# wangze22/StableDiffusion-PyTorch

Hardware: AMD Instinct MI355X
Metric: DDPM train steps/sec (cond-UNet, CelebHQ-256 latents, B=32) at 1/2/4/8 MI355X (higher is better)
Workload: dtype bf16; 1 GPU; cond-UNet celebhq_text_image_cond training step; model=cond-UNet 118.5M, global_batch=32, per_gpu_batch=32, parallelism=dp1

## Files before the change

### include/sdmi.h

```cpp
#ifndef SDMI_H
#define SDMI_H
#include <stdint.h>
#include <stddef.h>

#ifdef __cplusplus
extern "C" {
#endif

typedef void* sdmi_stream_t;

enum {
  SDMI_A_ROWMAJOR = 0,
  SDMI_A_CONV = 1,
  SDMI_A_COLMAJOR = 2
};
enum {
  SDMI_B_NK = 0,
  SDMI_B_KN = 1,
  SDMI_B_KN_CONV = 2
};

typedef struct sdmi_conv_geom {
  int ih, iw, cin, ldx;
  int kh, kw;
  int oh, ow;
  int sy, sx, oy0, ox0;
} sdmi_conv_geom;

typedef struct sdmi_gemm_desc {
  int m, n, k;
  int a_mode, b_mode;
  const void* a; int lda;
  const void* b; int ldb;
  sdmi_conv_geom geom;
  void* c; int ldc; int c_f32;
  const float* bias;
  const void* rowbias;
  int rb_ld, rb_div;
  const void* resid; int ldr;
  float alpha;
  int act;
  int remap, r_gh, r_gw, r_oh, r_ow, r_sy, r_sx, r_oy, r_ox;
  int perm, p_cin, p_taps, p_cvalid;
  int m_store, n_store;
  const void* a2; int lda2; int k_split;
  const float* bias2;
  int rb_mod;
  const void* aux; int ld_aux;
  int splits_hint;
  int tile_n_hint;
  float* sum_out;
  float* sum_out2;
  void* gsum_out;
  int gsum_ld;
  int sum_group;
  int variant_hint;
  const void* gn_x; int gn_ldx;
  const float* gn_tab;
  float* gn_part;
  int gn_P, gn_rb, gn_silu;
} sdmi_gemm_desc;

int sdmi_gemm_kernel_info(const sdmi_gemm_desc* d, int* variant, int* tile_n);
int sdmi_gemm_plan(const sdmi_gemm_desc* d, int* splits, size_t* workspace_bytes);
int sdmi_gemm(const sdmi_gemm_desc* d, void* workspace, size_t workspace_bytes, sdmi_stream_t stream);

#define SDMI_GEMM_GROUP_MAX 8
int sdmi_gemm_grouped_plan(const sdmi_gemm_desc* d, int ngroups, int* splits, size_t* workspace_bytes);
int sdmi_gemm_grouped(const sdmi_gemm_desc* d, int ngroups, void* workspace, size_t workspace_bytes,
                      sdmi_stream_t stream);

int sdmi_attn_fwd(const void* q, int ldq, const void* k, int ldk, const void* v, int ldv, void* out, int ldo,
                  float* lse, int B, int H, int N, int S, int d, sdmi_stream_t stream);
int sdmi_attn_bwd(const void* q, int ldq, const void* k, int ldk, const void* v, int ldv, const void* o, int ldo,
                  const void* dout, int lddo, const float* lse, float* delta_ws, void* dq, int lddq, void* dk,
                  int lddk, void* dv, int lddv, int B, int H, int N, int S, int d, sdmi_stream_t stream);
size_t sdmi_attn_bwd_workspace(int B, int H, int N, int S, int d);
int sdmi_attn_bwd_fused(const void* q, int ldq, const void* k, int ldk, const void* v, int ldv, const void* o, int ldo,
                        const void* dout, int lddo, const float* lse, float* delta_ws, void* ws, size_t ws_bytes,
                        void* dq, int lddq, void* dk, int lddk, void* dv, int lddv, int B, int H, int N, int S, int d,
                        sdmi_stream_t stream);

size_t sdmi_chan_reduce_workspace(int B, int P, int C);
int sdmi_gn_stats(const void* x, int ldx, int B, int P, int C, int G, float eps, const float* gamma, const float* beta,
                  float* ws, float* table, sdmi_stream_t stream);
int sdmi_gn_fwd(const void* x, int ldx, void* y, int ldy, int B, int P, int C, int G, float eps, const float* gamma,
                const float* beta, int silu, float* ws, float* table, sdmi_stream_t stream);
int sdmi_gn_apply(const void* x, int ldx, void* y, int ldy, const float* table, int B, int P, int C, int silu,
                  sdmi_stream_t stream);
int sdmi_gn_bwd(const void* x, int ldx, const void* dy, int lddy, void* dx, int lddx, const float* table,
                const float* gamma, int B, int P, int C, int G, int silu, float* ws, float* table2_ws, float* dgamma,
                float* dbeta, const void* addend, int ldadd, sdmi_stream_t stream);
int sdmi_gn_bwd_part(const void* x, int ldx, const void* dy, int lddy, void* dx, int lddx, const float* table,
                     const float* gamma, int B, int P, int C, int G, int silu, const float* part, int rb, float* ws,
                     float* dgamma, float* dbeta, const void* addend, int ldadd, sdmi_stream_t stream);

int sdmi_gn_bwd_rows(const void* x, int ldx, const void* dy, int lddy, void* dx, int lddx, const float* table,
                     const float* gamma, int B, int P, int C, int G, int silu, float* ws, float* table2_ws, float* rows,
                     const void* addend, int ldadd, sdmi_stream_t stream);
int sdmi_gn_bwd_part_rows(const void* x, int ldx, const void* dy, int lddy, void* dx, int lddx, const float* table,
                          const float* gamma, int B, int P, int C, int G, int silu, const float* part, int rb, float* ws,
                          float* rows, const void* addend, int ldadd, sdmi_stream_t stream);
int sdmi_gn_rows_sum(const float* rows, int B, int C, float* dgamma, float* dbeta, sdmi_stream_t stream);
#define SDMI_GN_ROWS_GROUP_MAX 16
typedef struct {
  const float* rows;
  float* dgamma;
  float* dbeta;
  int B, C;
} sdmi_gn_rows_job;
int sdmi_gn_rows_sum_grouped(const sdmi_gn_rows_job* jobs, int njobs, sdmi_stream_t stream);


int sdmi_chan_sum(const void* dy, int lddy, int B, int P, int C, float* ws, void* per_bc, int ld_bc, float* per_c,
                  float* per_c2, int c_store, sdmi_stream_t stream);

int sdmi_prep_input(const float* x, int B, int cx, int H, int W, const float* mask, int cmi, int MH, int MW,
                    const float* wcond, int cmo, void* out, int cpad, const float* keep, sdmi_stream_t stream);
int sdmi_cond_wgrad(const void* dxin, int ld, int cx, int B, int H, int W, const float* mask, int cmi, int MH, int MW,
                    int cmo, float* dw, const float* keep, sdmi_stream_t stream);
int sdmi_prep_input_cmap(const float* x, int B, int cx, int H, int W, const unsigned char* cmap, int cmi, int MH,
                         int MW, const float* wcond, int cmo, void* out, int cpad, const float* keep,
                         sdmi_stream_t stream);
int sdmi_cond_wgrad_cmap(const void* dxin, int ld, int cx, int B, int H, int W, const unsigned char* cmap, int cmi,
                         int MH, int MW, int cmo, float* dw, const float* keep, sdmi_stream_t stream);
int sdmi_nhwc_to_nchw(const void* src, int src_f32, int ld, int B, int C, int HW, float* dst, sdmi_stream_t stream);
int sdmi_nchw_to_nhwc_bf16(const float* src, int B, int C, int HW, void* dst, int ld, sdmi_stream_t stream);
int sdmi_add_noise(const float* x0, const float* eps, const long long* t, const float* sqrt_abar,
                   const float* sqrt_one_minus_abar, int B, long long per_sample, float* out, sdmi_stream_t stream);
size_t sdmi_mse_workspace(void);
int sdmi_mse(const float* pred, int ld, const float* target, int B, int C, int HW, float gscale,
             const float* gscale_dev, void* grad, float* ws, float* loss, sdmi_stream_t stream);
int sdmi_time_embedding(const long long* t, int tstride, int B, int dim, void* out, int ld, float* out_f32,
                        sdmi_stream_t stream);
int sdmi_silu(const void* x, const void* dy, void* y, long long n, sdmi_stream_t stream);
int sdmi_relu(const float* x, const float* dy, float* y, long long n, sdmi_stream_t stream);
int sdmi_copy_slice(const void* src, int lds, void* dst, int ldd, long long P, int C, int accumulate,
                    sdmi_stream_t stream);

int sdmi_ln_chunk_rows(int N);
int sdmi_ln_mod_fwd(const void* x, int ldx, const void* v, int ldv, const void* gate, void* xo, int ldxo,
                    const void* shift, const void* scale, int ld_mod, void* y, int ldy, float* mean, float* rstd,
                    int rows, int C, int N, float eps, int x_f32, sdmi_stream_t stream);
int sdmi_ln_mod_bwd(const void* x, int ldx, const float* mean, const float* rstd, const void* dy, int lddy,
                    const void* scale, int ld_mod, const void* dres, int lddres, void* dx, int lddx, float* psh,
                    float* psc, int ws_ld, const void* gate, const void* v, int ldv, void* dv, int lddv, float* pg,
                    int rows, int C, int N, int x_f32, void* dx16, int ld16, sdmi_stream_t stream);
int sdmi_mod_finalize(const float* ws, int B, int chunks, int ws_ld, int W, void* out, int ldo, sdmi_stream_t stream);
int sdmi_tokens_to_nchw(const void* src, int src_f32, int ld, int B, int C, int H, int W, int p, float* dst,
                        sdmi_stream_t stream);
int sdmi_nchw_to_tokens_bf16(const float* src, int B, int C, int H, int W, int p, void* dst, int ld,
                             sdmi_stream_t stream);
int sdmi_mse_patch(const float* pred, int ld, const float* target, int B, int C, int H, int W, int p, float gscale,
                   const float* gscale_dev, void* grad, float* ws, float* loss, sdmi_stream_t stream);

size_t sdmi_vq_workspace(long long pixels);
size_t sdmi_vq_bwd_workspace(void);
int sdmi_vq_bwd(const void* dzin, int ld_dzin, const float* zq, const float* w_post, const float* xq, const long long* idx,
                const float* codebook, int K, const float* z_enc, int ldz, const float* w_pre, int B, int HW, int C,
                float commitment_beta, float codebook_weight, void* dz_enc, int ld_out, float* ws, float* dw_post,
                float* db_post, float* dw_pre, float* db_pre, float* demb, const float* dzq_add, const float* loss_w,
                sdmi_stream_t stream);
int sdmi_vq_quantize(const float* z, int ldz, const float* w, const float* b, const float* codebook, int K, int B,
                     int HW, int C, float* zq, long long* idx, float* xq, float* ws, float* loss, sdmi_stream_t stream);
int sdmi_pointwise_in(const float* z, int B, int C, int HW, const float* w, const float* b, int cout, void* out,
                      int ld, sdmi_stream_t stream);

int sdmi_lpips_prep(const float* in0, int in0_nhwc, const float* in1, int in1_nhwc, int B, int H, int W,
                    const float* shift, const float* scale, int normalize, void* out, sdmi_stream_t stream);
int sdmi_lpips_image_grad(const void* d, int B, int H, int W, const float* scale, int normalize, float* out_nchw,
                          void* acc_nhwc, const float* mse_pred, const float* mse_target, sdmi_stream_t stream);
int sdmi_maxpool2_fwd(const void* x, int N, int H, int W, int C, void* y, sdmi_stream_t stream);
int sdmi_maxpool2_bwd(const void* x, const void* dy, int N, int H, int W, int C, void* dx, sdmi_stream_t stream);
size_t sdmi_lpips_dist_workspace(int B, int P, int C);
int sdmi_lpips_dist_fwd(const void* f, int ld, const float* w, int B, int P, int C, float* rn, float* ws, int accumulate,
                        float* val, sdmi_stream_t stream);
int sdmi_lpips_dist_bwd(const void* f, int ld, const float* w, const float* rn, const float* g, float gscale, int B,
                        int P, int C, int side, const void* addend, int ld_add, void* dy, int ld_dy,
                        sdmi_stream_t stream);
int sdmi_lpips_mean(const float* val, int B, float scale, float* out, sdmi_stream_t stream);

int sdmi_ddpm_prev(const float* xt, const float* eps, const float* z, long long n, long long* t_dev, const float* betas,
                   const float* alphas, const float* abar, const float* s1m, float* prev, float* x0, int decrement_t,
                   sdmi_stream_t stream);
int sdmi_ddim_prev(const float* xt, const float* eps, const float* noise, long long n, float alpha_t, float alpha_prev,
                   float eta, float* out, sdmi_stream_t stream);
int sdmi_ddim_prev_dev(const float* xt, const float* eps, const float* noise, long long n, const long long* ts,
                       const long long* tp, long long* idx, long long* t_dev, const float* abar, float eta, float* out,
                       int advance, sdmi_stream_t stream);
int sdmi_affine_step(const float* x, const float* eps, const float* z, long long n, float c1, float c2, float var,
                     float* out, sdmi_stream_t stream);
int sdmi_cfg_combine(const float* eps_cond, const float* eps_uncond, long long n, float scale, float* out,
                     sdmi_stream_t stream);
int sdmi_cfg_combine_nhwc(const void* pred, int src_f32, int ld, int B, int C, int HW, float scale, float* dst,
                          sdmi_stream_t stream);
int sdmi_ddpm_prev_dup(const float* xt, const float* eps, const float* z, long long n, long long* t_dev,
                       const float* betas, const float* alphas, const float* abar, const float* s1m, float* prev,
                       float* prev2, float* x0, int decrement_t, sdmi_stream_t stream);
int sdmi_ddim_prev_dev_dup(const float* xt, const float* eps, const float* noise, long long n, const long long* ts,
                           const long long* tp, long long* idx, long long* t_dev, const float* abar, float eta,
                           float* out, float* out2, int advance, sdmi_stream_t stream);

int sdmi_randn(float* out, long long n, unsigned long long seed, unsigned long long* offset_dev, int advance,
               sdmi_stream_t stream);

int sdmi_step_draw(float* noise, long long n, long long* t, int B, int T, const float* text, const float* empty,
                   float* txt, long long row_elems, float p_text, float* keep, float p_keep, unsigned long long seed,
                   unsigned long long offset, sdmi_stream_t stream);

typedef struct sdmi_pack_desc {
  const float* src;
  void* dst;
  long long so, si, skh, skw;
  int O, I, Ipad, KH, KW, kh_off, kh_mul, kw_off, kw_mul;
  int dst_ld;
} sdmi_pack_desc;
int sdmi_pack_chunk(void);
int sdmi_pack_weights(const sdmi_pack_desc* descs_dev, const void* bmap_dev, int nblocks, sdmi_stream_t stream);

typedef struct sdmi_tpack_desc {
  const void* src;
  void* dst;
  int O, I, taps;
  int src_ld, src_tap, dst_ld, dst_tap;
  signed char smap[16];
} sdmi_tpack_desc;
int sdmi_pack_transpose(const sdmi_tpack_desc* descs_dev, const void* bmap_dev, int nblocks, sdmi_stream_t stream);

size_t sdmi_optim_workspace(void);
int sdmi_clip_unscale(const float* grads, long long n, float max_norm, float* state, float* ws, int growth_interval,
                      int skip_if_loss_nonfinite, float grad_div, sdmi_stream_t stream);
size_t sdmi_optim_workspace_for(long long n);
int sdmi_clip_unscale_ws(const float* grads, long long n, float max_norm, float* state, float* ws, size_t ws_bytes,
                         int growth_interval, int skip_if_loss_nonfinite, float grad_div, sdmi_stream_t stream);
int sdmi_loss_flag(const float* src, float* dst, int mode, sdmi_stream_t stream);
int sdmi_clip_finalize(const float* partial, int n, float max_norm, float* state, int growth_interval,
                       int skip_if_loss_nonfinite, float grad_div, sdmi_stream_t stream);
int sdmi_adam_ema(float* params, const float* grads, float* m, float* v, float* ema, long long n, const float* state,
                  float lr, float b1, float b2, float eps, float ema_decay, float ema_alpha, sdmi_stream_t stream);
int sdmi_adam_ema_bf16(float* params, const float* grads, float* m, float* v, float* ema, long long n,
                       const float* state, float lr, float b1, float b2, float eps, float ema_decay, float ema_alpha,
                       void* params_bf16, sdmi_stream_t stream);
int sdmi_cast_bf16(const float* src, void* dst, long long n, sdmi_stream_t stream);

int sdmi_resize_nearest(const float* in, int BC, int IH, int IW, float* out, int OH, int OW, sdmi_stream_t stream);
int sdmi_chan_copy(const float* src, int src_c, int src_c0, float* dst, int dst_c, int dst_c0, int B, int C,
                   long long P, sdmi_stream_t stream);
int sdmi_modulate_fwd(const float* x, const float* r, const float* s, const float* t, int ls, float alpha, float* y,
                      int B, int N, int C, sdmi_stream_t stream);
int sdmi_modulate_bwd(const float* x, const float* dy, const float* s, int ls, float alpha, float* dx, float* ds,
                      float* dt, int B, int N, int C, sdmi_stream_t stream);
int sdmi_attn_map(const float* q, int ldq, const float* k, int ldk, int B, int H, int N, int S, int d, float scaling,
                  int average, float* out, sdmi_stream_t stream);


int sdmi_plan_begin(void);
int sdmi_plan_end(void** plan);
int sdmi_plan_recording(void);
int sdmi_plan_note_event(void* event, sdmi_stream_t stream);
int sdmi_plan_note_wait(sdmi_stream_t stream, void* event);
int sdmi_plan_note_callout(int id);
int sdmi_plan_info(const void* plan, int* ops, int* launches);
int sdmi_plan_replay(void* plan, int start, int* callout, int* next);
int sdmi_plan_destroy(void* plan);
int sdmi_plan_op_info(const void* plan, int i, int* kind, const char** name, int* grid, int* block, int* shmem);
int sdmi_plan_op_stream(const void* plan, int i, sdmi_stream_t* stream);
int sdmi_plan_time_op(void* plan, int i, int warm, int iters, float* us);

int sdmi_comm_load(const char* rccl_path);
int sdmi_comm_unique_id(unsigned char* id);
int sdmi_comm_init(const unsigned char* id, int nranks, int rank, void** comm);
int sdmi_allreduce(void* comm, void* buf, long long count, int dtype, sdmi_stream_t stream);
int sdmi_comm_destroy(void* comm);

#ifdef __cplusplus
}
#endif
#endif
```

### stablediffusion-pytorch_amd/csrc/plan.hip

```cpp
#include <cstring>
#include <memory>
#include <new>
#include <vector>

#include "../../include/sdmi.h"
#include "launch.h"

namespace sdmi_rt {

void* g_recording = nullptr;

namespace {

enum OpKind { OP_LAUNCH = 0, OP_EVENT = 1, OP_WAIT = 2, OP_CALLOUT = 3, OP_ALLREDUCE = 4 };

struct alignas(16) Chunk16 {
  unsigned char b[16];
};

struct Op {
  int kind;
  const void* fn = nullptr;
  dim3 grid, block;
  unsigned shmem = 0;
  hipStream_t stream = nullptr;
  hipEvent_t event = nullptr;
  int callout = -1;
  void* comm = nullptr;
  void* buf = nullptr;
  size_t count = 0;
  int dtype = 0;
  std::vector<Chunk16> args;
  std::vector<unsigned> offs;
};

struct Plan {
  std::vector<Op> ops;
  int launches = 0;
  std::vector<void*> scratch;
};

}

void record_launch(const void* fn, dim3 grid, dim3 block, unsigned shmem, hipStream_t stream, const void* args,
                   size_t bytes, const unsigned* offsets, int nargs) {
  Plan* p = (Plan*)g_recording;
  Op op;
  op.kind = OP_LAUNCH;
  op.fn = fn;
  op.grid = grid;
  op.block = block;
  op.shmem = shmem;
  op.stream = stream;
  op.args.resize((bytes + 15) / 16);
  if (bytes) memcpy(op.args.data(), args, bytes);
  op.offs.assign(offsets, offsets + nargs);
  if ((int)p->scratch.size() < nargs) p->scratch.resize(nargs);
  p->ops.push_back(std::move(op));
  ++p->launches;
}

void record_allreduce(void* comm, void* buf, size_t count, int dtype, hipStream_t stream) {
  Plan* p = (Plan*)g_recording;
  Op op;
  op.kind = OP_ALLREDUCE;
  op.comm = comm;
  op.buf = buf;
  op.count = count;
  op.dtype = dtype;
  op.stream = stream;
  p->ops.push_back(std::move(op));
}

}

using sdmi_rt::Plan;

extern "C" int sdmi_plan_begin(void) {
  if (sdmi_rt::g_recording) return -1;
  sdmi_rt::g_recording = new (std::nothrow) Plan();
  return sdmi_rt::g_recording ? 0 : -2;
}

extern "C" int sdmi_plan_end(void** plan) {
  if (!plan || !sdmi_rt::g_recording) return -1;
  *plan = sdmi_rt::g_recording;
  sdmi_rt::g_recording = nullptr;
  return 0;
}

extern "C" int sdmi_plan_recording(void) { return sdmi_rt::g_recording != nullptr; }

extern "C" int sdmi_plan_note_event(void* event, sdmi_stream_t stream) {
  Plan* p = (Plan*)sdmi_rt::g_recording;
  if (!p) return 0;
  if (!event) return -1;
  sdmi_rt::Op op;
  op.kind = sdmi_rt::OP_EVENT;
  op.event = (hipEvent_t)event;
  op.stream = (hipStream_t)stream;
  p->ops.push_back(std::move(op));
  return 0;
}

extern "C" int sdmi_plan_note_wait(sdmi_stream_t stream, void* event) {
  Plan* p = (Plan*)sdmi_rt::g_recording;
  if (!p) return 0;
  if (!event) return -1;
  sdmi_rt::Op op;
  op.kind = sdmi_rt::OP_WAIT;
  op.event = (hipEvent_t)event;
  op.stream = (hipStream_t)stream;
  p->ops.push_back(std::move(op));
  return 0;
}

extern "C" int sdmi_plan_note_callout(int id) {
  Plan* p = (Plan*)sdmi_rt::g_recording;
  if (!p) return 0;
  sdmi_rt::Op op;
  op.kind = sdmi_rt::OP_CALLOUT;
  op.callout = id;
  p->ops.push_back(std::move(op));
  return 0;
}

extern "C" int sdmi_plan_info(const void* plan, int* ops, int* launches) {
  const Plan* p = (const Plan*)plan;
  if (!p) return -1;
  if (ops) *ops = (int)p->ops.size();
  if (launches) *launches = p->launches;
  return 0;
}

extern "C" int sdmi_plan_replay(void* plan, int start, int* callout, int* next) {
  Plan* p = (Plan*)plan;
  if (!p || start < 0 || !callout || !next) return -1;
  void** ptrs = p->scratch.data();
  const int n = (int)p->ops.size();
  for (int i = start; i < n; ++i) {
    const sdmi_rt::Op& op = p->ops[i];
    hipError_t e = hipSuccess;
    switch (op.kind) {
      case sdmi_rt::OP_LAUNCH: {
        const unsigned char* base = (const unsigned char*)op.args.data();
        for (size_t a = 0; a < op.offs.size(); ++a) ptrs[a] = (void*)(base + op.offs[a]);
        e = hipLaunchKernel(op.fn, op.grid, op.block, ptrs, op.shmem, op.stream);
        break;
      }
      case sdmi_rt::OP_EVENT: e = hipEventRecord(op.event, op.stream); break;
      case sdmi_rt::OP_WAIT: e = hipStreamWaitEvent(op.stream, op.event, 0); break;
      case sdmi_rt::OP_ALLREDUCE: {
        const int rc = sdmi_rt::issue_allreduce(op.comm, op.buf, op.count, op.dtype, op.stream);
        if (rc != 0) {
          *callout = -1;
          *next = i;
          return rc;
        }
        break;
      }
      default:
        *callout = op.callout;
        *next = i + 1;
        return 0;
    }
    if (e != hipSuccess) {
      *callout = -1;
      *next = i;
      return (int)e;
    }
  }
  *callout = -1;
  *next = n;
  return 0;
}

extern "C" int sdmi_plan_op_stream(const void* plan, int i, sdmi_stream_t* stream) {
  const Plan* p = (const Plan*)plan;
  if (!p || i < 0 || i >= (int)p->ops.size() || !stream) return -1;
  *stream = (sdmi_stream_t)p->ops[i].stream;
  return 0;
}

extern "C" int sdmi_plan_op_info(const void* plan, int i, int* kind, const char** name, int* grid, int* block,
                                 int* shmem) {
  const Plan* p = (const Plan*)plan;
  if (!p || i < 0 || i >= (int)p->ops.size()) return -1;
  const sdmi_rt::Op& op = p->ops[i];
  if (kind) *kind = op.kind;
  if (name) *name = op.kind == sdmi_rt::OP_LAUNCH ? hipKernelNameRefByPtr(op.fn, op.stream) : nullptr;
  if (grid) {
    grid[0] = (int)op.grid.x;
    grid[1] = (int)op.grid.y;
    grid[2] = (int)op.grid.z;
  }
  if (block) *block = (int)(op.block.x * op.block.y * op.block.z);
  if (shmem) *shmem = (int)op.shmem;
  return 0;
}

extern "C" int sdmi_plan_time_op(void* plan, int i, int warm, int iters, float* us) {
  Plan* p = (Plan*)plan;
  if (!p || i < 0 || i >= (int)p->ops.size() || iters < 1 || !us) return -1;
  const sdmi_rt::Op& op = p->ops[i];
  if (op.kind != sdmi_rt::OP_LAUNCH) return -2;
  void** ptrs = p->scratch.data();
  const unsigned char* base = (const unsigned char*)op.args.data();
  for (size_t a = 0; a < op.offs.size(); ++a) ptrs[a] = (void*)(base + op.offs[a]);
  hipEvent_t e0, e1;
  if (hipEventCreate(&e0) != hipSuccess) return -3;
  if (hipEventCreate(&e1) != hipSuccess) return -3;
  hipError_t e = hipSuccess;
  for (int w = 0; w < warm && e == hipSuccess; ++w) e = hipLaunchKernel(op.fn, op.grid, op.block, ptrs, op.shmem, op.stream);
  if (e == hipSuccess) e = hipEventRecord(e0, op.stream);
  for (int r = 0; r < iters && e == hipSuccess; ++r) e = hipLaunchKernel(op.fn, op.grid, op.block, ptrs, op.shmem, op.stream);
  if (e == hipSuccess) e = hipEventRecord(e1, op.stream);
  if (e == hipSuccess) e = hipEventSynchronize(e1);
  float ms = 0.f;
  if (e == hipSuccess) e = hipEventElapsedTime(&ms, e0, e1);
  (void)hipEventDestroy(e0);
  (void)hipEventDestroy(e1);
  if (e != hipSuccess) return (int)e;
  *us = ms * 1000.f / (float)iters;
  return 0;
}

extern "C" int sdmi_plan_destroy(void* plan) {
  delete (Plan*)plan;
  return 0;
}
```

### stablediffusion-pytorch_amd/sdmi/_lib.py

```python
import ctypes
import os

_HERE = os.path.dirname(os.path.abspath(__file__))
DEFAULT_LIB_PATH = os.path.join(_HERE, "libsdmi.so")
LIB_PATH = os.environ.get("SDMI_LIB_PATH") or DEFAULT_LIB_PATH

A_ROWMAJOR, A_CONV, A_COLMAJOR = 0, 1, 2
B_NK, B_KN, B_KN_CONV = 0, 1, 2


class ConvGeom(ctypes.Structure):
    _fields_ = [(n, ctypes.c_int) for n in
                ("ih", "iw", "cin", "ldx", "kh", "kw", "oh", "ow", "sy", "sx", "oy0", "ox0")]


class GemmDesc(ctypes.Structure):
    _fields_ = [
        ("m", ctypes.c_int), ("n", ctypes.c_int), ("k", ctypes.c_int),
        ("a_mode", ctypes.c_int), ("b_mode", ctypes.c_int),
        ("a", ctypes.c_void_p), ("lda", ctypes.c_int),
        ("b", ctypes.c_void_p), ("ldb", ctypes.c_int),
        ("geom", ConvGeom),
        ("c", ctypes.c_void_p), ("ldc", ctypes.c_int), ("c_f32", ctypes.c_int),
        ("bias", ctypes.c_void_p),
        ("rowbias", ctypes.c_void_p), ("rb_ld", ctypes.c_int), ("rb_div", ctypes.c_int),
        ("resid", ctypes.c_void_p), ("ldr", ctypes.c_int),
        ("alpha", ctypes.c_float),
        ("act", ctypes.c_int),
        ("remap", ctypes.c_int), ("r_gh", ctypes.c_int), ("r_gw", ctypes.c_int),
        ("r_oh", ctypes.c_int), ("r_ow", ctypes.c_int), ("r_sy", ctypes.c_int), ("r_sx", ctypes.c_int),
        ("r_oy", ctypes.c_int), ("r_ox", ctypes.c_int),
        ("perm", ctypes.c_int), ("p_cin", ctypes.c_int), ("p_taps", ctypes.c_int), ("p_cvalid", ctypes.c_int),
        ("m_store", ctypes.c_int), ("n_store", ctypes.c_int),
        ("a2", ctypes.c_void_p), ("lda2", ctypes.c_int), ("k_split", ctypes.c_int),
        ("bias2", ctypes.c_void_p),
        ("rb_mod", ctypes.c_int),
        ("aux", ctypes.c_void_p), ("ld_aux", ctypes.c_int),
        ("splits_hint", ctypes.c_int),
        ("tile_n_hint", ctypes.c_int),
        ("sum_out", ctypes.c_void_p), ("sum_out2", ctypes.c_void_p), ("gsum_out", ctypes.c_void_p),
        ("gsum_ld", ctypes.c_int), ("sum_group", ctypes.c_int),
        ("variant_hint", ctypes.c_int),
        ("gn_x", ctypes.c_void_p), ("gn_ldx", ctypes.c_int),
        ("gn_tab", ctypes.c_void_p),
        ("gn_part", ctypes.c_void_p),
        ("gn_P", ctypes.c_int), ("gn_rb", ctypes.c_int), ("gn_silu", ctypes.c_int),
    ]


_lib = None

_P, _I, _F, _L = ctypes.c_void_p, ctypes.c_int, ctypes.c_float, ctypes.c_longlong
_SZ = ctypes.c_size_t


class GnRowsJob(ctypes.Structure):
    _fields_ = [("rows", ctypes.c_void_p), ("dgamma", ctypes.c_void_p), ("dbeta", ctypes.c_void_p),
                ("B", ctypes.c_int), ("C", ctypes.c_int)]


GN_ROWS_GROUP_MAX = 16


class TPackDesc(ctypes.Structure):
    _fields_ = [("src", ctypes.c_void_p), ("dst", ctypes.c_void_p)] + [(n, ctypes.c_int) for n in (
        "O", "I", "taps", "src_ld", "src_tap", "dst_ld", "dst_tap")] + [("smap", ctypes.c_byte * 16)]


class PackDesc(ctypes.Structure):
    _fields_ = [("src", ctypes.c_void_p), ("dst", ctypes.c_void_p),
                ("so", ctypes.c_longlong), ("si", ctypes.c_longlong), ("skh", ctypes.c_longlong),
                ("skw", ctypes.c_longlong)] + [(n, ctypes.c_int) for n in
                                                ("O", "I", "Ipad", "KH", "KW", "kh_off", "kh_mul", "kw_off", "kw_mul",
                                                 "dst_ld")]


SIGNATURES = {
    "sdmi_gemm_plan": ([ctypes.POINTER(GemmDesc), ctypes.POINTER(ctypes.c_int), ctypes.POINTER(ctypes.c_size_t)], _I),
    "sdmi_gemm": ([ctypes.POINTER(GemmDesc), _P, _SZ, _P], _I),
    "sdmi_gemm_grouped_plan": ([ctypes.POINTER(GemmDesc), _I, ctypes.POINTER(ctypes.c_int),
                                ctypes.POINTER(ctypes.c_size_t)], _I),
    "sdmi_gemm_grouped": ([ctypes.POINTER(GemmDesc), _I, _P, _SZ, _P], _I),
    "sdmi_gemm_kernel_info": ([ctypes.POINTER(GemmDesc), ctypes.POINTER(ctypes.c_int), ctypes.POINTER(ctypes.c_int)],
                              _I),
    "sdmi_attn_fwd": ([_P, _I, _P, _I, _P, _I, _P, _I, _P, _I, _I, _I, _I, _I, _P], _I),
    "sdmi_attn_bwd": ([_P, _I, _P, _I, _P, _I, _P, _I, _P, _I, _P, _P, _P, _I, _P, _I, _P, _I,
                       _I, _I, _I, _I, _I, _P], _I),
    "sdmi_attn_bwd_workspace": ([_I, _I, _I, _I, _I], _SZ),
    "sdmi_attn_bwd_fused": ([_P, _I, _P, _I, _P, _I, _P, _I, _P, _I, _P, _P, _P, _SZ, _P, _I, _P, _I, _P, _I,
                             _I, _I, _I, _I, _I, _P], _I),
    "sdmi_chan_reduce_workspace": ([_I, _I, _I], _SZ),
    "sdmi_gn_stats": ([_P, _I, _I, _I, _I, _I, _F, _P, _P, _P, _P, _P], _I),
    "sdmi_gn_apply": ([_P, _I, _P, _I, _P, _I, _I, _I, _I, _P], _I),
    "sdmi_gn_fwd": ([_P, _I, _P, _I, _I, _I, _I, _I, _F, _P, _P, _I, _P, _P, _P], _I),
    "sdmi_gn_bwd": ([_P, _I, _P, _I, _P, _I, _P, _P, _I, _I, _I, _I, _I, _P, _P, _P, _P, _P, _I, _P], _I),
    "sdmi_gn_bwd_part": ([_P, _I, _P, _I, _P, _I, _P, _P, _I, _I, _I, _I, _I, _P, _I, _P, _P, _P, _P, _I, _P], _I),
    "sdmi_gn_bwd_rows": ([_P, _I, _P, _I, _P, _I, _P, _P, _I, _I, _I, _I, _I, _P, _P, _P, _P, _I, _P], _I),
    "sdmi_gn_bwd_part_rows": ([_P, _I, _P, _I, _P, _I, _P, _P, _I, _I, _I, _I, _I, _P, _I, _P, _P, _P, _I, _P], _I),
    "sdmi_gn_rows_sum": ([_P, _I, _I, _P, _P, _P], _I),
    "sdmi_gn_rows_sum_grouped": ([_P, _I, _P], _I),
    "sdmi_chan_sum": ([_P, _I, _I, _I, _I, _P, _P, _I, _P, _P, _I, _P], _I),
    "sdmi_prep_input": ([_P, _I, _I, _I, _I, _P, _I, _I, _I, _P, _I, _P, _I, _P, _P], _I),
    "sdmi_cond_wgrad": ([_P, _I, _I, _I, _I, _I, _P, _I, _I, _I, _I, _P, _P, _P], _I),
    "sdmi_prep_input_cmap": ([_P, _I, _I, _I, _I, _P, _I, _I, _I, _P, _I, _P, _I, _P, _P], _I),
    "sdmi_cond_wgrad_cmap": ([_P, _I, _I, _I, _I, _I, _P, _I, _I, _I, _I, _P, _P, _P], _I),
    "sdmi_nhwc_to_nchw": ([_P, _I, _I, _I, _I, _I, _P, _P], _I),
    "sdmi_nchw_to_nhwc_bf16": ([_P, _I, _I, _I, _P, _I, _P], _I),
    "sdmi_add_noise": ([_P, _P, _P, _P, _P, _I, _L, _P, _P], _I),
    "sdmi_mse_workspace": ([], _SZ),
    "sdmi_mse": ([_P, _I, _P, _I, _I, _I, _F, _P, _P, _P, _P, _P], _I),
    "sdmi_time_embedding": ([_P, _I, _I, _I, _P, _I, _P, _P], _I),
    "sdmi_silu": ([_P, _P, _P, _L, _P], _I),
    "sdmi_copy_slice": ([_P, _I, _P, _I, _L, _I, _I, _P], _I),
    "sdmi_pack_chunk": ([], _I),
    "sdmi_pack_weights": ([_P, _P, _I, _P], _I),
    "sdmi_pack_transpose": ([_P, _P, _I, _P], _I),
    "sdmi_optim_workspace": ([], _SZ),
    "sdmi_clip_unscale": ([_P, _L, _F, _P, _P, _I, _I, _F, _P], _I),
    "sdmi_optim_workspace_for": ([_L], _SZ),
    "sdmi_clip_unscale_ws": ([_P, _L, _F, _P, _P, _SZ, _I, _I, _F, _P], _I),
    "sdmi_loss_flag": ([_P, _P, _I, _P], _I),
    "sdmi_clip_finalize": ([_P, _I, _F, _P, _I, _I, _F, _P], _I),
    "sdmi_norm_block": ([], _L),
    "sdmi_sumsq_blocks": ([_P, _L, _P, _P], _I),
    "sdmi_widen_bf16_sumsq": ([_P, _P, _L, _P, _P], _I),
    "sdmi_adam_ema": ([_P, _P, _P, _P, _P, _L, _P, _F, _F, _F, _F, _F, _F, _P], _I),
    "sdmi_adam_ema_bf16": ([_P, _P, _P, _P, _P, _L, _P, _F, _F, _F, _F, _F, _F, _P, _P], _I),
    "sdmi_cast_bf16": ([_P, _P, _L, _P], _I),
    "sdmi_resize_nearest": ([_P, _I, _I, _I, _P, _I, _I, _P], _I),
    "sdmi_chan_copy": ([_P, _I, _I, _P, _I, _I, _I, _I, _L, _P], _I),
    "sdmi_modulate_fwd": ([_P, _P, _P, _P, _I, _F, _P, _I, _I, _I, _P], _I),
    "sdmi_modulate_bwd": ([_P, _P, _P, _I, _F, _P, _P, _P, _I, _I, _I, _P], _I),
    "sdmi_attn_map": ([_P, _I, _P, _I, _I, _I, _I, _I, _I, _F, _I, _P, _P], _I),
    "sdmi_ln_chunk_rows": ([_I], _I),
    "sdmi_ln_mod_fwd": ([_P, _I, _P, _I, _P, _P, _I, _P, _P, _I, _P, _I, _P, _P, _I, _I, _I, _F, _I, _P], _I),
    "sdmi_ln_mod_bwd": ([_P, _I, _P, _P, _P, _I, _P, _I, _P, _I, _P, _I, _P, _P, _I, _P, _P, _I, _P, _I, _P,
                         _I, _I, _I, _I, _P, _I, _P], _I),
    "sdmi_mod_finalize": ([_P, _I, _I, _I, _I, _P, _I, _P], _I),
    "sdmi_tokens_to_nchw": ([_P, _I, _I, _I, _I, _I, _I, _I, _P, _P], _I),
    "sdmi_nchw_to_tokens_bf16": ([_P, _I, _I, _I, _I, _I, _P, _I, _P], _I),
    "sdmi_vq_workspace": ([_L], _SZ),
    "sdmi_vq_quantize": ([_P, _I, _P, _P, _P, _I, _I, _I, _I, _P, _P, _P, _P, _P, _P], _I),
    "sdmi_pointwise_in": ([_P, _I, _I, _I, _P, _P, _I, _P, _I, _P], _I),
    "sdmi_ddpm_prev": ([_P, _P, _P, _L, _P, _P, _P, _P, _P, _P, _P, _I, _P], _I),
    "sdmi_ddim_prev": ([_P, _P, _P, _L, _F, _F, _F, _P, _P], _I),
    "sdmi_ddim_prev_dev": ([_P, _P, _P, _L, _P, _P, _P, _P, _P, _F, _P, _I, _P], _I),
    "sdmi_affine_step": ([_P, _P, _P, _L, _F, _F, _F, _P, _P], _I),
    "sdmi_cfg_combine": ([_P, _P, _L, _F, _P, _P], _I),
    "sdmi_cfg_combine_nhwc": ([_P, _I, _I, _I, _I, _I, _F, _P, _P], _I),
    "sdmi_ddpm_prev_dup": ([_P, _P, _P, _L, _P, _P, _P, _P, _P, _P, _P, _P, _I, _P], _I),
    "sdmi_ddim_prev_dev_dup": ([_P, _P, _P, _L, _P, _P, _P, _P, _P, _F, _P, _P, _I, _P], _I),
    "sdmi_mse_patch": ([_P, _I, _P, _I, _I, _I, _I, _I, _F, _P, _P, _P, _P, _P], _I),
    "sdmi_randn": ([_P, _L, ctypes.c_ulonglong, _P, _I, _P], _I),
    "sdmi_step_draw": ([_P, _L, _P, _I, _I, _P, _P, _P, _L, ctypes.c_float, _P, ctypes.c_float, ctypes.c_ulonglong,
                        ctypes.c_ulonglong, _P], _I),
    "sdmi_relu": ([_P, _P, _P, _L, _P], _I),
    "sdmi_vq_bwd_workspace": ([], _SZ),
    "sdmi_vq_bwd": ([_P, _I, _P, _P, _P, _P, _P, _I, _P, _I, _P, _I, _I, _I, _F, _F, _P, _I, _P, _P, _P, _P, _P, _P,
                     _P, _P, _P], _I),
    "sdmi_lpips_prep": ([_P, _I, _P, _I, _I, _I, _I, _P, _P, _I, _P, _P], _I),
    "sdmi_lpips_image_grad": ([_P, _I, _I, _I, _P, _I, _P, _P, _P, _P, _P], _I),
    "sdmi_maxpool2_fwd": ([_P, _I, _I, _I, _I, _P, _P], _I),
    "sdmi_maxpool2_bwd": ([_P, _P, _I, _I, _I, _I, _P, _P], _I),
    "sdmi_lpips_dist_workspace": ([_I, _I, _I], _SZ),
    "sdmi_lpips_dist_fwd": ([_P, _I, _P, _I, _I, _I, _P, _P, _I, _P, _P], _I),
    "sdmi_lpips_dist_bwd": ([_P, _I, _P, _P, _P, _F, _I, _I, _I, _I, _P, _I, _P, _I, _P], _I),
    "sdmi_lpips_mean": ([_P, _I, _F, _P, _P], _I),
    "sdmi_plan_begin": ([], _I),
    "sdmi_plan_end": ([ctypes.POINTER(ctypes.c_void_p)], _I),
    "sdmi_plan_recording": ([], _I),
    "sdmi_plan_note_event": ([_P, _P], _I),
    "sdmi_plan_note_wait": ([_P, _P], _I),
    "sdmi_plan_note_callout": ([_I], _I),
    "sdmi_plan_info": ([_P, ctypes.POINTER(ctypes.c_int), ctypes.POINTER(ctypes.c_int)], _I),
    "sdmi_plan_replay": ([_P, _I, ctypes.POINTER(ctypes.c_int), ctypes.POINTER(ctypes.c_int)], _I),
    "sdmi_plan_destroy": ([_P], _I),
    "sdmi_plan_op_stream": ([_P, _I, ctypes.POINTER(ctypes.c_void_p)], _I),
    "sdmi_plan_op_info": ([_P, _I, ctypes.POINTER(ctypes.c_int), ctypes.POINTER(ctypes.c_char_p),
                           ctypes.POINTER(ctypes.c_int), ctypes.POINTER(ctypes.c_int), ctypes.POINTER(ctypes.c_int)], _I),
    "sdmi_plan_time_op": ([_P, _I, _I, _I, ctypes.POINTER(ctypes.c_float)], _I),
    "sdmi_comm_load": ([ctypes.c_char_p], _I),
    "sdmi_comm_unique_id": ([_P], _I),
    "sdmi_comm_init": ([_P, _I, _I, ctypes.POINTER(ctypes.c_void_p)], _I),
    "sdmi_allreduce": ([_P, _P, _L, _I, _P], _I),
    "sdmi_comm_destroy": ([_P], _I),
}


class _Lib:

    def __init__(self, cdll):
        self._cdll = cdll
        ab = bool(os.environ.get("SDMI_LIB_PATH"))
        for name, (argt, rest) in SIGNATURES.items():
            if ab and not hasattr(cdll, name):
                continue
            fn = getattr(cdll, name)
            fn.argtypes = argt
            fn.restype = rest
            setattr(self, name, fn)


def lib():
    global _lib
    if _lib is None:
        if not os.path.exists(LIB_PATH):
            raise RuntimeError(f"libsdmi.so not built ({LIB_PATH}); run __graft_entry__.build()")
        import torch
        if os.path.abspath(LIB_PATH) != DEFAULT_LIB_PATH:
            import sys
            print(f"sdmi: SDMI_LIB_PATH override in effect, loading {LIB_PATH} (A/B timing only)", file=sys.stderr)
        _lib = _Lib(ctypes.CDLL(LIB_PATH))
    return _lib


class SdmiError(RuntimeError):
    pass


def check(rc, what):
    if rc != 0:
        raise SdmiError(f"{what} failed with status {rc}")
```

### stablediffusion-pytorch_amd/sdmi/plan.py

```python
import ctypes

import torch

RECORDING = None
KEEP = None


def _lib():
    from . import _lib as L
    return L.lib()


def record(fn, *args):
    r = fn(*args)
    if RECORDING is not None:
        RECORDING.append((fn, args))
        _check(_lib().sdmi_plan_note_callout(len(RECORDING) - 1), "sdmi_plan_note_callout")
    return r


def _check(rc, what):
    if rc != 0:
        raise RuntimeError(f"{what} failed with status {rc}")


def as_operand(t, dtype=torch.float32):
    if t.dtype == dtype and t.is_contiguous():
        return t
    out = torch.empty(t.shape, dtype=dtype, device=t.device)
    record(out.copy_, t)
    return out


def timesteps(t, device):
    if isinstance(t, torch.Tensor) and t.device == torch.device(device) and t.dtype == torch.int64 and t.is_contiguous():
        return t.reshape(-1)
    if isinstance(t, torch.Tensor) and t.device.type == "cuda":
        return as_operand(t.reshape(-1), torch.int64)
    return torch.as_tensor(t, device=device).long().reshape(-1)


def record_event(ev, stream):
    ev.record(stream)
    if RECORDING is not None:
        KEEP.append(ev)
        _check(_lib().sdmi_plan_note_event(ev.cuda_event, stream.cuda_stream), "sdmi_plan_note_event")


def wait_event(stream, ev):
    stream.wait_event(ev)
    if RECORDING is not None:
        KEEP.append(ev)
        _check(_lib().sdmi_plan_note_wait(stream.cuda_stream, ev.cuda_event), "sdmi_plan_note_wait")


def wait_stream(dst, src):
    if RECORDING is None:
        dst.wait_stream(src)
        return
    ev = torch.cuda.Event()
    record_event(ev, src)
    wait_event(dst, ev)


class StepPlan:
    def __init__(self, step_fn, device=None):
        global RECORDING, KEEP
        self.device = torch.device(device) if device is not None else torch.device("cuda", torch.cuda.current_device())
        torch.cuda.synchronize(self.device)
        self.pool = torch.cuda.MemPool()
        lib = _lib()
        self.handle = None
        ops, keep = [], []
        with torch.cuda.use_mem_pool(self.pool, device=self.device):
            _check(lib.sdmi_plan_begin(), "sdmi_plan_begin")
            RECORDING, KEEP = ops, keep
            h = ctypes.c_void_p()
            try:
                step_fn()
            finally:
                RECORDING, KEEP = None, None
                _check(lib.sdmi_plan_end(ctypes.byref(h)), "sdmi_plan_end")
                self.handle = h
        torch.cuda.synchronize(self.device)
        self.ops = ops
        self.keep = keep
        self._cid, self._next = ctypes.c_int(0), ctypes.c_int(0)

    def info(self):
        n, k = ctypes.c_int(0), ctypes.c_int(0)
        _check(_lib().sdmi_plan_info(self.handle, ctypes.byref(n), ctypes.byref(k)), "sdmi_plan_info")
        return n.value, k.value, len(self.ops)

    def __len__(self):
        return self.info()[0]

    def collectives(self):
        lib = _lib()
        n, kind = self.info()[0], ctypes.c_int(0)
        native = 0
        for i in range(n):
            _check(lib.sdmi_plan_op_info(self.handle, i, ctypes.byref(kind), None, None, None, None), "sdmi_plan_op_info")
            native += kind.value == 4
        return native + sum(1 for fn, _ in self.ops if getattr(fn, "__name__", "") == "_issue")

    def replay(self):
        lib = _lib()
        cid, nxt = self._cid, self._next
        pos = 0
        while True:
            rc = lib.sdmi_plan_replay(self.handle, pos, ctypes.byref(cid), ctypes.byref(nxt))
            if rc != 0:
                raise RuntimeError(f"plan replay failed at op {nxt.value} with status {rc}")
            if cid.value < 0:
                return
            fn, args = self.ops[cid.value]
            fn(*args)
            pos = nxt.value

    def __del__(self):
        if getattr(self, "handle", None) is not None and self.handle.value:
            try:
                _lib().sdmi_plan_destroy(self.handle)
            except Exception:
                pass
            self.handle = None
```

Before: 78.96 steps/s.

## Compile recorded plan cross-stream edges: fold, alias, and drop redundant waits

Adds a compile pass over the recorded step plan that tracks cross-stream dependencies with vector clocks. It folds event records into the preceding kernel launch via hipExtLaunchKernel's completion event, aliases duplicate back-to-back events, and drops waits already implied by earlier ones. Plan-owned events can also skip the system fence when no allreduce stream consumes them. The aim is fewer host API calls and GPU-side sync packets per replayed step, at the cost of a complex dependency analysis that could drop a required ordering if it has a bug.

```diff
diff --git a/include/sdmi.h b/include/sdmi.h
--- a/include/sdmi.h
+++ b/include/sdmi.h
@@ -266,6 +266,12 @@
 int sdmi_plan_op_info(const void* plan, int i, int* kind, const char** name, int* grid, int* block, int* shmem);
 int sdmi_plan_op_stream(const void* plan, int i, sdmi_stream_t* stream);
 int sdmi_plan_time_op(void* plan, int i, int warm, int iters, float* us);
+int sdmi_plan_note_edge(sdmi_stream_t src, sdmi_stream_t dst);
+int sdmi_plan_edge_info(const void* plan, int* recorded, int* compiled, int* folded, int* aliased, int* waits_dropped,
+                        int* owned_events);
+int sdmi_plan_op_edge(const void* plan, int i, int* event, int* owned, int* fate);
+int sdmi_plan_set_edges(int mode);
+int sdmi_plan_edge_probe(int variant, int nofence, int k, int chain, size_t bytes, int reps, float* span_us);
 
 int sdmi_comm_load(const char* rccl_path);
 int sdmi_comm_unique_id(unsigned char* id);
diff --git a/stablediffusion-pytorch_amd/csrc/plan.hip b/stablediffusion-pytorch_amd/csrc/plan.hip
--- a/stablediffusion-pytorch_amd/csrc/plan.hip
+++ b/stablediffusion-pytorch_amd/csrc/plan.hip
@@ -1,10 +1,15 @@
+#include <hip/hip_ext.h>
+
+#include <cstdlib>
 #include <cstring>
+#include <map>
 #include <memory>
 #include <new>
 #include <vector>
 
 #include "../../include/sdmi.h"
 #include "launch.h"
+#include "plan_edges.h"
 
 namespace sdmi_rt {
 
@@ -25,6 +30,7 @@
   unsigned shmem = 0;
   hipStream_t stream = nullptr;
   hipEvent_t event = nullptr;
+  int eid = -1;
   int callout = -1;
   void* comm = nullptr;
   void* buf = nullptr;
@@ -34,11 +40,91 @@
   std::vector<unsigned> offs;
 };
 
+struct CompiledOp {
+  int src;
+  hipEvent_t event;
+};
+
 struct Plan {
   std::vector<Op> ops;
   int launches = 0;
   std::vector<void*> scratch;
+  std::map<hipEvent_t, int> event_ids;
+  int nevents = 0;
+  std::vector<char> owned;
+  std::vector<hipEvent_t> plain, fast;
+  std::vector<CompiledOp> compiled[2];
+  std::vector<int> fate;
+  sdmi_edges::Stats stats;
+  int mode = 1;
+
+  ~Plan() {
+    for (hipEvent_t e : plain)
+      if (e) (void)hipEventDestroy(e);
+    for (hipEvent_t e : fast)
+      if (e) (void)hipEventDestroy(e);
+  }
 };
+
+int initial_edges() {
+  const char* v = getenv("SDMI_PLAN_EDGES");
+  return v && v[0] >= '0' && v[0] <= '2' && !v[1] ? v[0] - '0' : 1;
+}
+int g_edges = initial_edges();
+constexpr int kDefaultList = 0;
+
+int event_id(Plan* p, hipEvent_t ev) {
+  auto it = p->event_ids.find(ev);
+  if (it != p->event_ids.end()) return it->second;
+  p->event_ids[ev] = p->nevents;
+  p->owned.push_back(0);
+  return p->nevents++;
+}
+
+hipEvent_t handle(const Plan* p, const Op& op, bool fast) {
+  return op.event ? op.event : (fast ? p->fast : p->plain)[op.eid];
+}
+
+int compile_plan(Plan* p) {
+  std::map<hipStream_t, int> sid;
+  std::vector<sdmi_edges::Rec> recs;
+  recs.reserve(p->ops.size());
+  for (const Op& op : p->ops) {
+    sdmi_edges::Rec r;
+    r.kind = op.kind;
+    r.stream = -1;
+    if (op.kind != OP_CALLOUT) r.stream = sid.emplace(op.stream, (int)sid.size()).first->second;
+    r.event = op.eid;
+    r.owned = op.eid >= 0 && p->owned[op.eid];
+    recs.push_back(r);
+  }
+  p->plain.assign(p->nevents, nullptr);
+  p->fast.assign(p->nevents, nullptr);
+  for (int v = 0; v < 2; ++v) {
+    const sdmi_edges::Result res = sdmi_edges::compile(recs, v == 0);
+    if (v == 0) {
+      for (int e = 0; e < p->nevents; ++e) {
+        if (!p->owned[e]) continue;
+        const unsigned flags = hipEventDisableTiming | (res.system_fence[e] ? 0u : (unsigned)hipEventDisableSystemFence);
+        if (hipEventCreateWithFlags(&p->plain[e], hipEventDisableTiming) != hipSuccess) return -3;
+        if (hipEventCreateWithFlags(&p->fast[e], flags) != hipSuccess) return -3;
+      }
+    }
+    if (v == kDefaultList) {
+      p->fate = res.fate;
+      p->stats = res.stats;
+    }
+    std::vector<Op*> by_event(p->nevents, nullptr);
+    for (Op& op : p->ops)
+      if (op.eid >= 0) by_event[op.eid] = &op;
+    for (const sdmi_edges::COp& c : res.ops) {
+      CompiledOp co{c.src, nullptr};
+      if (c.event >= 0) co.event = handle(p, *by_event[c.event], true);
+      p->compiled[v].push_back(co);
+    }
+  }
+  return 0;
+}
 
 }
 
@@ -86,7 +172,7 @@
   if (!plan || !sdmi_rt::g_recording) return -1;
   *plan = sdmi_rt::g_recording;
   sdmi_rt::g_recording = nullptr;
-  return 0;
+  return sdmi_rt::compile_plan((Plan*)*plan);
 }
 
 extern "C" int sdmi_plan_recording(void) { return sdmi_rt::g_recording != nullptr; }
@@ -98,6 +184,7 @@
   sdmi_rt::Op op;
   op.kind = sdmi_rt::OP_EVENT;
   op.event = (hipEvent_t)event;
+  op.eid = sdmi_rt::event_id(p, op.event);
   op.stream = (hipStream_t)stream;
   p->ops.push_back(std::move(op));
   return 0;
@@ -110,8 +197,25 @@
   sdmi_rt::Op op;
   op.kind = sdmi_rt::OP_WAIT;
   op.event = (hipEvent_t)event;
+  op.eid = sdmi_rt::event_id(p, op.event);
   op.stream = (hipStream_t)stream;
   p->ops.push_back(std::move(op));
+  return 0;
+}
+
+extern "C" int sdmi_plan_note_edge(sdmi_stream_t src, sdmi_stream_t dst) {
+  Plan* p = (Plan*)sdmi_rt::g_recording;
+  if (!p) return 0;
+  const int eid = p->nevents++;
+  p->owned.push_back(1);
+  sdmi_rt::Op rec, wait;
+  rec.kind = sdmi_rt::OP_EVENT;
+  rec.stream = (hipStream_t)src;
+  wait.kind = sdmi_rt::OP_WAIT;
+  wait.stream = (hipStream_t)dst;
+  rec.eid = wait.eid = eid;
+  p->ops.push_back(std::move(rec));
+  p->ops.push_back(std::move(wait));
   return 0;
 }
 
@@ -133,23 +237,60 @@
   return 0;
 }
 
+extern "C" int sdmi_plan_edge_info(const void* plan, int* recorded, int* compiled, int* folded, int* aliased,
+                                   int* waits_dropped, int* owned_events) {
+  const Plan* p = (const Plan*)plan;
+  if (!p) return -1;
+  if (recorded) *recorded = p->stats.recorded;
+  if (compiled) *compiled = p->stats.compiled;
+  if (folded) *folded = p->stats.folded;
+  if (aliased) *aliased = p->stats.aliased;
+  if (waits_dropped) *waits_dropped = p->stats.waits_dropped;
+  if (owned_events) *owned_events = p->stats.owned_events;
+  return 0;
+}
+
+extern "C" int sdmi_plan_op_edge(const void* plan, int i, int* event, int* owned, int* fate) {
+  const Plan* p = (const Plan*)plan;
+  if (!p || i < 0 || i >= (int)p->ops.size()) return -1;
+  const sdmi_rt::Op& op = p->ops[i];
+  if (op.eid < 0) return -2;
+  if (event) *event = op.eid;
+  if (owned) *owned = p->owned[op.eid];
+  if (fate) *fate = p->fate[i];
+  return 0;
+}
+
+extern "C" int sdmi_plan_set_edges(int mode) {
+  if (mode < 0 || mode > 2) return -1;
+  sdmi_rt::g_edges = mode;
+  return 0;
+}
+
 extern "C" int sdmi_plan_replay(void* plan, int start, int* callout, int* next) {
   Plan* p = (Plan*)plan;
   if (!p || start < 0 || !callout || !next) return -1;
+  if (start == 0) p->mode = sdmi_rt::g_edges;
   void** ptrs = p->scratch.data();
-  const int n = (int)p->ops.size();
+  const bool verbatim = p->mode == 0;
+  const std::vector<sdmi_rt::CompiledOp>& list = p->compiled[p->mode == 2 ? 1 : sdmi_rt::kDefaultList];
+  const int n = verbatim ? (int)p->ops.size() : (int)list.size();
   for (int i = start; i < n; ++i) {
-    const sdmi_rt::Op& op = p->ops[i];
+    const sdmi_rt::Op& op = p->ops[verbatim ? i : list[i].src];
+    const hipEvent_t ev = verbatim ? (op.eid >= 0 ? sdmi_rt::handle(p, op, false) : nullptr) : list[i].event;
     hipError_t e = hipSuccess;
     switch (op.kind) {
       case sdmi_rt::OP_LAUNCH: {
         const unsigned char* base = (const unsigned char*)op.args.data();
         for (size_t a = 0; a < op.offs.size(); ++a) ptrs[a] = (void*)(base + op.offs[a]);
-        e = hipLaunchKernel(op.fn, op.grid, op.block, ptrs, op.shmem, op.stream);
+        if (ev)
+          e = hipExtLaunchKernel(op.fn, op.grid, op.block, ptrs, op.shmem, op.stream, nullptr, ev, 0);
+        else
+          e = hipLaunchKernel(op.fn, op.grid, op.block, ptrs, op.shmem, op.stream);
         break;
       }
-      case sdmi_rt::OP_EVENT: e = hipEventRecord(op.event, op.stream); break;
-      case sdmi_rt::OP_WAIT: e = hipStreamWaitEvent(op.stream, op.event, 0); break;
+      case sdmi_rt::OP_EVENT: e = hipEventRecord(ev, op.stream); break;
+      case sdmi_rt::OP_WAIT: e = hipStreamWaitEvent(op.stream, ev, 0); break;
       case sdmi_rt::OP_ALLREDUCE: {
         const int rc = sdmi_rt::issue_allreduce(op.comm, op.buf, op.count, op.dtype, op.stream);
         if (rc != 0) {
@@ -225,6 +366,78 @@
   return 0;
 }
 
+namespace {
+
+__global__ void edge_probe_kernel(float* p, size_t n) {
+  const size_t i = (size_t)blockIdx.x * blockDim.x + threadIdx.x;
+  if (i < n) p[i] = p[i] * 0.5f + 1.0f;
+}
+
+}
+
+extern "C" int sdmi_plan_edge_probe(int variant, int nofence, int k, int chain, size_t bytes, int reps, float* span_us) {
+  if (variant < 0 || variant > 5 || chain < 1 || chain > 4096 || k < 1 || k > 64 || reps < 1 || bytes < 4 ||
+      bytes > ((size_t)256 << 20) || !span_us)
+    return -1;
+  const size_t n = bytes / 4, nb = 4096;
+  const int nev = variant == 3 ? chain * k : chain;
+  hipStream_t A = nullptr, B = nullptr;
+  float *bufA = nullptr, *bufB = nullptr;
+  hipEvent_t t0 = nullptr, t1 = nullptr;
+  std::vector<hipEvent_t> evs(nev, nullptr);
+  hipError_t e = hipStreamCreateWithFlags(&A, hipStreamNonBlocking);
+  if (e == hipSuccess) e = hipStreamCreateWithFlags(&B, hipStreamNonBlocking);
+  if (e == hipSuccess) e = hipMalloc((void**)&bufA, n * 4);
+  if (e == hipSuccess) e = hipMalloc((void**)&bufB, nb * 4);
+  if (e == hipSuccess) e = hipMemsetAsync(bufA, 0, n * 4, A);
+  if (e == hipSuccess) e = hipMemsetAsync(bufB, 0, nb * 4, B);
+  if (e == hipSuccess) e = hipEventCreate(&t0);
+  if (e == hipSuccess) e = hipEventCreate(&t1);
+  const unsigned flags = hipEventDisableTiming | (nofence ? (unsigned)hipEventDisableSystemFence : 0u);
+  for (int i = 0; i < nev && e == hipSuccess; ++i) e = hipEventCreateWithFlags(&evs[i], flags);
+  if (variant == 3)
+    for (int i = 0; i < nev && e == hipSuccess; ++i) e = hipEventRecord(evs[i], B);
+  if (e == hipSuccess) e = hipDeviceSynchronize();
+  const dim3 block(256), grid((unsigned)((n + 255) / 256)), gridB((unsigned)((nb + 255) / 256));
+  void* argsA[2] = {(void*)&bufA, (void*)&n};
+  void* argsB[2] = {(void*)&bufB, (void*)&nb};
+  float total = 0.f;
+  for (int r = 0; r <= reps && e == hipSuccess; ++r) {
+    e = hipEventRecord(t0, A);
+    for (int i = 0; i < chain && e == hipSuccess; ++i) {
+      if (variant == 3)
+        for (int w = 0; w < k && e == hipSuccess; ++w) e = hipStreamWaitEvent(A, evs[i * k + w], 0);
+      if (e != hipSuccess) break;
+      if (variant == 2)
+        e = hipExtLaunchKernel((const void*)edge_probe_kernel, grid, block, argsA, 0, A, nullptr, evs[i], 0);
+      else
+        e = hipLaunchKernel((const void*)edge_probe_kernel, grid, block, argsA, 0, A);
+      if (e == hipSuccess && (variant == 1 || variant >= 4)) e = hipEventRecord(evs[i], A);
+      if (e == hipSuccess && (variant == 1 || variant == 2 || variant == 5)) {
+        e = hipStreamWaitEvent(B, evs[i], 0);
+        if (e == hipSuccess && variant != 5) e = hipLaunchKernel((const void*)edge_probe_kernel, gridB, block, argsB, 0, B);
+      }
+    }
+    if (e == hipSuccess) e = hipEventRecord(t1, A);
+    if (e == hipSuccess) e = hipDeviceSynchronize();
+    float ms = 0.f;
+    if (e == hipSuccess) e = hipEventElapsedTime(&ms, t0, t1);
+    if (r > 0) total += ms;
+  }
+  if (e != hipSuccess) (void)hipDeviceSynchronize();
+  for (hipEvent_t ev : evs)
+    if (ev) (void)hipEventDestroy(ev);
+  if (t0) (void)hipEventDestroy(t0);
+  if (t1) (void)hipEventDestroy(t1);
+  if (bufA) (void)hipFree(bufA);
+  if (bufB) (void)hipFree(bufB);
+  if (A) (void)hipStreamDestroy(A);
+  if (B) (void)hipStreamDestroy(B);
+  if (e != hipSuccess) return (int)e;
+  *span_us = total * 1000.f / (float)reps;
+  return 0;
+}
+
 extern "C" int sdmi_plan_destroy(void* plan) {
   delete (Plan*)plan;
   return 0;
diff --git a/stablediffusion-pytorch_amd/csrc/plan_edges.h b/stablediffusion-pytorch_amd/csrc/plan_edges.h
--- /dev/null
+++ b/stablediffusion-pytorch_amd/csrc/plan_edges.h
@@ -0,0 +1,208 @@
+#pragma once
+#include <algorithm>
+#include <vector>
+
+namespace sdmi_edges {
+
+enum Kind { LAUNCH = 0, EVENT = 1, WAIT = 2, CALLOUT = 3, ALLREDUCE = 4 };
+enum Fate { KEPT = 0, FOLDED = 1, ALIASED = 2, DROPPED = 3 };
+
+struct Rec {
+  int kind;
+  int stream;
+  int event;
+  bool owned;
+};
+
+struct COp {
+  int src;
+  int event;
+};
+
+struct Stats {
+  int recorded = 0, compiled = 0, folded = 0, aliased = 0, waits_dropped = 0, owned_events = 0;
+};
+
+struct Result {
+  std::vector<COp> ops;
+  std::vector<int> fate;
+  std::vector<char> system_fence;
+  Stats stats;
+};
+
+inline Result compile(const std::vector<Rec>& recs, bool fold) {
+  const int n = (int)recs.size();
+  int S = 0, E = 0;
+  bool any_callout = false;
+  for (const Rec& r : recs) {
+    S = std::max(S, r.stream + 1);
+    E = std::max(E, r.event + 1);
+    any_callout |= r.kind == CALLOUT;
+  }
+  Result out;
+  out.fate.assign(n, KEPT);
+  out.stats.recorded = n;
+  std::vector<char> owned(E, 0), has_allreduce(S, 0);
+  std::vector<int> last_rec(E, -1);
+  for (int i = 0; i < n; ++i) {
+    const Rec& r = recs[i];
+    if (r.kind == EVENT) last_rec[r.event] = i;
+    if ((r.kind == EVENT || r.kind == WAIT) && r.owned) owned[r.event] = 1;
+    if (r.kind == ALLREDUCE) has_allreduce[r.stream] = 1;
+  }
+  for (int e = 0; e < E; ++e) out.stats.owned_events += owned[e];
+
+  typedef std::vector<int> Clock;
+  enum EvState { CARRIED = 0, VALID = 1, OPAQUE = 2 };
+  std::vector<int> cnt(S, 0);
+  std::vector<Clock> clock(S, Clock(2 * S, 0));
+  std::vector<Clock> snap(E);
+  std::vector<int> state(E, CARRIED), alias(E);
+  for (int e = 0; e < E; ++e) {
+    alias[e] = e;
+    if (last_rec[e] < 0) state[e] = OPAQUE;
+  }
+  struct Pending {
+    int cidx;
+    Clock cap;
+    int src, ord;
+  };
+  std::vector<std::vector<Pending>> cluster(S);
+  std::vector<int> dup_event(S, -1);
+  std::vector<int> last_op(S, -1);
+  std::vector<int> last_wait(E, -1);
+  std::vector<int> last_seen_rec(E, -1);
+  std::vector<std::vector<int>> carried(S, std::vector<int>(S, -1));
+  std::vector<std::vector<char>> consumers(E, std::vector<char>(S, 0));
+  int last_callout = -1;
+  std::vector<char> dead;
+
+  auto emit = [&](int src, int event) {
+    out.ops.push_back(COp{src, event});
+    dead.push_back(0);
+    return (int)out.ops.size() - 1;
+  };
+  std::vector<int> cidx_of(n, -1);
+
+  for (int i = 0; i < n; ++i) {
+    const Rec& r = recs[i];
+    switch (r.kind) {
+      case LAUNCH:
+      case ALLREDUCE:
+        ++cnt[r.stream];
+        cluster[r.stream].clear();
+        dup_event[r.stream] = -1;
+        cidx_of[i] = emit(i, -1);
+        break;
+      case CALLOUT:
+        for (int s = 0; s < S; ++s) {
+          ++cnt[s];
+          cluster[s].clear();
+          dup_event[s] = -1;
+          std::fill(carried[s].begin(), carried[s].end(), -1);
+        }
+        for (int e = 0; e < E; ++e)
+          if (!owned[e]) state[e] = OPAQUE;
+        last_callout = i;
+        emit(i, -1);
+        break;
+      case EVENT: {
+        const int s = r.stream, e = r.event;
+        cluster[s].clear();
+        if (owned[e] && dup_event[s] >= 0) {
+          alias[e] = dup_event[s];
+          out.fate[i] = ALIASED;
+          ++out.stats.aliased;
+          break;
+        }
+        alias[e] = e;
+        snap[e] = clock[s];
+        snap[e][s] = cnt[s] + 1;
+        state[e] = VALID;
+        const int j = last_op[s];
+        if (fold && j >= 0 && recs[j].kind == LAUNCH && out.ops[cidx_of[j]].event < 0 && last_wait[e] < j &&
+            last_seen_rec[e] < j && last_callout < j) {
+          out.ops[cidx_of[j]].event = e;
+          out.fate[i] = FOLDED;
+          ++out.stats.folded;
+        } else {
+          emit(i, e);
+        }
+        last_seen_rec[e] = i;
+        dup_event[s] = owned[e] ? e : -1;
+        break;
+      }
+      case WAIT: {
+        const int d = r.stream, e = alias[r.event];
+        last_wait[r.event] = i;
+        last_wait[e] = i;
+        consumers[e][d] = 1;
+        dup_event[d] = -1;
+        Pending p;
+        p.src = -1;
+        p.ord = -1;
+        bool drop = false;
+        if (state[e] == VALID) {
+          const Clock& cap = snap[e];
+          bool covered = true;
+          for (int s = 0; s < 2 * S && covered; ++s) covered = cap[s] <= (s == d ? cnt[d] + 1 : clock[d][s]);
+          if (covered) {
+            drop = true;
+          } else {
+            for (int s = 0; s < 2 * S; ++s) clock[d][s] = std::max(clock[d][s], cap[s]);
+            for (Pending& q : cluster[d]) {
+              if (q.cap.empty() || dead[q.cidx]) continue;
+              bool le = true;
+              for (int s = 0; s < 2 * S && le; ++s) le = q.cap[s] <= cap[s];
+              if (le) dead[q.cidx] = 1;
+            }
+            p.cap = cap;
+          }
+        } else if (state[e] == CARRIED) {
+          const int src = recs[last_rec[e]].stream, ord = last_rec[e];
+          if (carried[d][src] >= ord) {
+            drop = true;
+          } else {
+            carried[d][src] = ord;
+            for (Pending& q : cluster[d])
+              if (q.src == src && q.ord <= ord && !dead[q.cidx]) dead[q.cidx] = 1;
+            p.src = src;
+            p.ord = ord;
+          }
+        }
+        if (drop) {
+          out.fate[i] = DROPPED;
+          ++out.stats.waits_dropped;
+        } else {
+          if (state[e] != VALID) ++clock[d][S + d];
+          p.cidx = emit(i, e);
+          cluster[d].push_back(p);
+        }
+        break;
+      }
+    }
+    if (r.stream >= 0) last_op[r.stream] = i;
+  }
+  std::vector<COp> kept;
+  kept.reserve(out.ops.size());
+  for (size_t c = 0; c < out.ops.size(); ++c) {
+    if (dead[c]) {
+      out.fate[out.ops[c].src] = DROPPED;
+      ++out.stats.waits_dropped;
+    } else {
+      kept.push_back(out.ops[c]);
+    }
+  }
+  out.ops.swap(kept);
+  out.stats.compiled = (int)out.ops.size();
+  out.system_fence.assign(E, 1);
+  for (int e = 0; e < E; ++e) {
+    if (!owned[e] || any_callout) continue;
+    bool fence = false;
+    for (int s = 0; s < S; ++s) fence |= consumers[e][s] && has_allreduce[s];
+    out.system_fence[e] = fence ? 1 : 0;
+  }
+  return out;
+}
+
+}
diff --git a/stablediffusion-pytorch_amd/sdmi/_lib.py b/stablediffusion-pytorch_amd/sdmi/_lib.py
--- a/stablediffusion-pytorch_amd/sdmi/_lib.py
+++ b/stablediffusion-pytorch_amd/sdmi/_lib.py
@@ -179,6 +179,11 @@
     "sdmi_plan_op_info": ([_P, _I, ctypes.POINTER(ctypes.c_int), ctypes.POINTER(ctypes.c_char_p),
                            ctypes.POINTER(ctypes.c_int), ctypes.POINTER(ctypes.c_int), ctypes.POINTER(ctypes.c_int)], _I),
     "sdmi_plan_time_op": ([_P, _I, _I, _I, ctypes.POINTER(ctypes.c_float)], _I),
+    "sdmi_plan_note_edge": ([_P, _P], _I),
+    "sdmi_plan_edge_info": ([_P] + [ctypes.POINTER(ctypes.c_int)] * 6, _I),
+    "sdmi_plan_op_edge": ([_P, _I] + [ctypes.POINTER(ctypes.c_int)] * 3, _I),
+    "sdmi_plan_set_edges": ([_I], _I),
+    "sdmi_plan_edge_probe": ([_I, _I, _I, _I, _SZ, _I, ctypes.POINTER(ctypes.c_float)], _I),
     "sdmi_comm_load": ([ctypes.c_char_p], _I),
     "sdmi_comm_unique_id": ([_P], _I),
     "sdmi_comm_init": ([_P, _I, _I, ctypes.POINTER(ctypes.c_void_p)], _I),
diff --git a/stablediffusion-pytorch_amd/sdmi/plan.py b/stablediffusion-pytorch_amd/sdmi/plan.py
--- a/stablediffusion-pytorch_amd/sdmi/plan.py
+++ b/stablediffusion-pytorch_amd/sdmi/plan.py
@@ -55,12 +55,9 @@
 
 
 def wait_stream(dst, src):
-    if RECORDING is None:
-        dst.wait_stream(src)
-        return
-    ev = torch.cuda.Event()
-    record_event(ev, src)
-    wait_event(dst, ev)
+    dst.wait_stream(src)
+    if RECORDING is not None:
+        _check(_lib().sdmi_plan_note_edge(src.cuda_stream, dst.cuda_stream), "sdmi_plan_note_edge")
 
 
 class StepPlan:
@@ -91,6 +88,12 @@
         n, k = ctypes.c_int(0), ctypes.c_int(0)
         _check(_lib().sdmi_plan_info(self.handle, ctypes.byref(n), ctypes.byref(k)), "sdmi_plan_info")
         return n.value, k.value, len(self.ops)
+
+    def edge_info(self):
+        v = [ctypes.c_int(0) for _ in range(6)]
+        _check(_lib().sdmi_plan_edge_info(self.handle, *[ctypes.byref(x) for x in v]), "sdmi_plan_edge_info")
+        return dict(zip(("recorded", "compiled", "folded", "aliased", "waits_dropped", "owned_events"),
+                        (x.value for x in v)))
 
     def __len__(self):
         return self.info()[0]
```

Result: faster. 80.76 steps/s, median of 6 (+2.3%).
